# yang-song/score_sde_pytorch

Measured on NVIDIA H100. Metric: PC-sampler images/sec, NCSN++ CIFAR-10 1000-step VE, higher is better.
Workload: dtype f16 operands (11-bit significand, as tf32), f32 accumulate and activations

## Files before the change

### include/scoresde_b200.h

```cpp
#ifndef SCORESDE_B200_H_
#define SCORESDE_B200_H_

#ifdef __cplusplus
extern "C" {
#endif

#define B200_API __attribute__((visibility("default")))

B200_API const char* b200_last_error(void);
B200_API int b200_version(void);
B200_API int b200_device_sm_count(int* out);

B200_API int b200_upfirdn2d_f32(const float* x, const float* kernel_host, float* y,
                                int major, int in_h, int in_w, int minor, int kh, int kw,
                                int up_x, int up_y, int down_x, int down_y,
                                int pad_x0, int pad_x1, int pad_y0, int pad_y1, void* stream);

B200_API int b200_fused_bias_act_f32(const float* x, const float* b, const float* ref, float* y,
                                     long long n, int step_b, int size_b, int act, int grad,
                                     float alpha, float scale, void* stream);

B200_API int b200_groupnorm_nhwc_f32(const float* x1, int c1, const float* x2, int c2,
                                     const float* gamma, const float* beta, int batch, int hw, int groups,
                                     float eps, int silu, int round_tf32,
                                     float* stats_ws ,
                                     float* y, float* raw_or_null, void* stream);
B200_API int b200_softmax_rows_f32(const float* s, float* p, long long rows, int t, float scale,
                                   int round_tf32, void* stream);
B200_API int b200_randn_like_torch_f32(float* out, long long numel, unsigned long long seed,
                                       unsigned long long offset, unsigned long long* offset_inc_out,
                                       unsigned long long* offset_ws_dev , void* stream);

B200_API int b200_conv_nhwc_f32(const float* x1, int c1, const float* x2, int c2, int batch, int h, int w,
                                const float* w_packed, const float* bias, int c_out, int ksize,
                                const float* rowvec, long long rowvec_ld, const float* residual, float scale,
                                int round_tf32, float* out, int impl, void* stream);
B200_API int b200_conv_skip_nhwc_f32(const float* x, int c, const float* s1, int cs1, const float* s2, int cs2,
                                     int batch, int h, int w, const float* w_packed, const float* bias,
                                     const float* w_skip, const float* bias_skip, int c_out, const float* residual,
                                     float scale, int round_tf32, float* out, void* stream);
B200_API int b200_pack_conv_weight_f32(const float* w_oihw, float* w_packed, int c_out, int c_in, int ksize,
                                       int round_tf32, void* stream);
B200_API int b200_attention_core_f32(const float* qk, const float* vT, const float* w3, const float* bv,
                                     const float* b3, const float* x, float* out, double* qstats, int nimg,
                                     int t, int c, float out_scale, int operand_f16, void* stream);
B200_API int b200_gemm_nt_f32(const float* a, long long lda, int a_batch_rows, const float* w, long long ldw,
                              int w_batch_rows, int nbatch, int m, int n, int k, const float* bias,
                              int round_tf32, float* out, long long ldo, int impl, void* stream);

typedef struct b200_ncsnpp b200_ncsnpp_t;

typedef struct {
  int image_size, num_channels, nf, num_res_blocks;
  int num_levels;  int ch_mult[8];
  int num_attn_resolutions;  int attn_resolutions[8];
  int centered, scale_by_sigma, skip_rescale, conditional;
  int progressive_input;
  int fir_taps;  float fir_kernel[8];
  int precision;
  int keep_activations;
  int lanes;
  int cuda_core_head;
  int separate_groupnorm;
  int embedding_type;
  int naive_resample;
  int progressive;
  int pdl;
  int no_halo;
// ... 83 lines not shown
```

### score_sde_pytorch_b200/_lib.py

```python
import ctypes
import os
import threading

from . import build as _build

_LOCK = threading.Lock()
_LIB = None

c_void_p, c_int, c_ll, c_ull, c_float = (ctypes.c_void_p, ctypes.c_int, ctypes.c_longlong,
                                         ctypes.c_ulonglong, ctypes.c_float)
c_char_p = ctypes.c_char_p
P = ctypes.POINTER


class NcsnppConfig(ctypes.Structure):
  _fields_ = [('image_size', c_int), ('num_channels', c_int), ('nf', c_int), ('num_res_blocks', c_int),
              ('num_levels', c_int), ('ch_mult', c_int * 8),
              ('num_attn_resolutions', c_int), ('attn_resolutions', c_int * 8),
              ('centered', c_int), ('scale_by_sigma', c_int), ('skip_rescale', c_int), ('conditional', c_int),
              ('progressive_input', c_int),
              ('fir_taps', c_int), ('fir_kernel', c_float * 8),
              ('precision', c_int), ('keep_activations', c_int), ('lanes', c_int),
              ('cuda_core_head', c_int), ('separate_groupnorm', c_int),
              ('embedding_type', c_int), ('naive_resample', c_int), ('progressive', c_int), ('pdl', c_int),
# ... 7 lines not shown
              ('pa', P(c_float)), ('pb', P(c_float)), ('pc', P(c_float)),
              ('ca', P(c_float)), ('cb', P(c_float)), ('cc', P(c_float)),
              ('constraint', c_int), ('cm', P(c_float)), ('cs', P(c_float)),
              ('color_m', c_float * 9), ('color_minv', c_float * 9), ('noise_nhwc', c_int)]


SIGNATURES = {
  'b200_last_error': (c_char_p, []),
  'b200_version': (c_int, []),
  'b200_device_sm_count': (c_int, [P(c_int)]),
  'b200_upfirdn2d_f32': (c_int, [c_void_p, P(c_float), c_void_p] + [c_int] * 14 + [c_void_p]),
  'b200_fused_bias_act_f32': (c_int, [c_void_p, c_void_p, c_void_p, c_void_p, c_ll, c_int, c_int, c_int, c_int,
                                      c_float, c_float, c_void_p]),
  'b200_groupnorm_nhwc_f32': (c_int, [c_void_p, c_int, c_void_p, c_int, c_void_p, c_void_p, c_int, c_int, c_int,
                                      c_float, c_int, c_int, c_void_p, c_void_p, c_void_p, c_void_p]),
  'b200_softmax_rows_f32': (c_int, [c_void_p, c_void_p, c_ll, c_int, c_float, c_int, c_void_p]),
  'b200_randn_like_torch_f32': (c_int, [c_void_p, c_ll, c_ull, c_ull, P(c_ull), c_void_p, c_void_p]),
  'b200_conv_nhwc_f32': (c_int, [c_void_p, c_int, c_void_p, c_int, c_int, c_int, c_int, c_void_p, c_void_p, c_int,
                                 c_int, c_void_p, c_ll, c_void_p, c_float, c_int, c_void_p, c_int, c_void_p]),
  'b200_conv_skip_nhwc_f32': (c_int, [c_void_p, c_int, c_void_p, c_int, c_void_p, c_int, c_int, c_int, c_int, c_void_p,
                                      c_void_p, c_void_p, c_void_p, c_int, c_void_p, c_float, c_int, c_void_p, c_void_p]),
  'b200_attention_core_f32': (c_int, [c_void_p, c_void_p, c_void_p, c_void_p, c_void_p, c_void_p, c_void_p, c_void_p,
                                      c_int, c_int, c_int, c_float, c_int, c_void_p]),
  'b200_pack_conv_weight_f32': (c_int, [c_void_p, c_void_p, c_int, c_int, c_int, c_int, c_void_p]),
  'b200_gemm_nt_f32': (c_int, [c_void_p, c_ll, c_int, c_void_p, c_ll, c_int, c_int, c_int, c_int, c_int, c_void_p,
                               c_int, c_void_p, c_ll, c_int, c_void_p]),
  'b200_ncsnpp_create': (c_int, [P(NcsnppConfig), P(c_void_p)]),
  'b200_ncsnpp_destroy': (None, [c_void_p]),
  'b200_ncsnpp_num_params': (c_int, [c_void_p]),
  'b200_ncsnpp_param_info': (c_int, [c_void_p, c_int, c_char_p, c_int, P(c_ll), P(c_int)]),
  'b200_ncsnpp_weights_bytes': (c_ll, [c_void_p]),
  'b200_ncsnpp_bind_weights': (c_int, [c_void_p, c_void_p]),
  'b200_ncsnpp_load_param': (c_int, [c_void_p, c_int, c_void_p, c_void_p]),
  'b200_ncsnpp_num_ops': (c_ll, [c_void_p]),
  'b200_ncsnpp_op_info': (c_int, [c_void_p, c_ll, c_char_p, c_int, P(c_int), P(ctypes.c_double)]),
  'b200_ncsnpp_op_bytes': (c_int, [c_void_p, c_ll, P(ctypes.c_double)]),
  'b200_ncsnpp_profile_ops': (c_int, [c_void_p, c_void_p, c_void_p, c_int, c_void_p, c_void_p, c_void_p, c_ll]),
  'b200_ncsnpp_workspace_bytes': (c_ll, [c_void_p, c_int]),
  'b200_ncsnpp_bind_workspace': (c_int, [c_void_p, c_int, c_void_p, c_ll]),
  'b200_ncsnpp_forward': (c_int, [c_void_p, c_void_p, c_void_p, c_int, c_void_p, c_void_p]),
  'b200_ncsnpp_tap': (c_int, [c_void_p, c_int, c_void_p, c_ll, P(c_int), c_void_p]),
  'b200_ncsnpp_launches_per_forward': (c_ll, [c_void_p]),
  'b200_ncsnpp_jvp': (c_int, [c_void_p, c_void_p, c_void_p, c_int, c_void_p, c_void_p, c_void_p, c_void_p]),
  'b200_ncsnpp_tap_tangent': (c_int, [c_void_p, c_int, c_void_p, c_ll, P(c_int), c_void_p]),
  'b200_ncsnpp_profile_forward': (c_int, [c_void_p, c_void_p, c_void_p, c_int, c_void_p, c_void_p,
                                          P(c_float), P(ctypes.c_double), P(c_ll)]),
# ... 60 lines not shown
```

### score_sde_pytorch_b200/csrc/api.cu

```cuda
#include "kernels.h"
#include "../../include/scoresde_b200.h"
#include <cstring>

namespace b200 {
namespace { thread_local bool tl_pdl = false; }
bool pdl_active() { return tl_pdl; }
PdlScope::PdlScope(bool on) : prev(tl_pdl) { tl_pdl = on; }
PdlScope::~PdlScope() { tl_pdl = prev; }


static thread_local char g_err[1024] = "";

void set_error(const char* fmt, ...) {
  va_list ap;
  va_start(ap, fmt);
  vsnprintf(g_err, sizeof(g_err), fmt, ap);
  va_end(ap);
}
const char* last_error() { return g_err; }

}

using namespace b200;

// ... 107 lines not shown
  d.a3 = s1; d.C3 = cs1; d.a4 = s2; d.C4 = s2 ? cs2 : 0; d.w2 = w_skip;
  d.epi = ep;
  TcGemmPlan* pl = nullptr;
  if (int r = tc_gemm_plan_create(d, &pl)) return r;
  const int r = tc_gemm_launch(pl, static_cast<cudaStream_t>(stream));
  tc_gemm_plan_destroy(pl);
  return r;
}

int b200_attention_core_f32(const float* qk, const float* vT, const float* w3, const float* bv, const float* b3,
                            const float* x, float* out, double* qstats, int nimg, int t, int c, float out_scale,
                            int operand_f16, void* stream) {
  B200_REQUIRE(tc_attn_supported(t, c), "attention_core: only T=256, C=256 is implemented (got T=%d C=%d)", t, c);
  TcAttnDesc d; memset(&d, 0, sizeof(d));
  d.qk = qk; d.vT = vT; d.w3 = w3; d.bv = bv; d.b3 = b3; d.x = x; d.out = out; d.qstats = qstats;
  d.nimg = nimg; d.T = t; d.C = c; d.out_scale = out_scale; d.f16 = operand_f16 ? 1 : 0;
  TcAttnPlan* pl = nullptr;
  if (int r = tc_attn_plan_create(d, &pl)) return r;
  const int r = tc_attn_launch(pl, static_cast<cudaStream_t>(stream));
  tc_attn_plan_destroy(pl);
  return r;
}

int b200_gemm_nt_f32(const float* a, long long lda, int a_batch_rows, const float* w, long long ldw, int w_batch_rows,
                     int nbatch, int m, int n, int k, const float* bias, int round_tf32, float* out, long long ldo,
                     int impl, void* stream) {
  B200_REQUIRE(a && w && out && nbatch > 0, "gemm_nt: bad argument");
  cudaStream_t st = static_cast<cudaStream_t>(stream);
  Epilogue ep; memset(&ep, 0, sizeof(ep));
  ep.bias = bias; ep.scale = 1.f; ep.round_tf32 = round_tf32; ep.rows_per_img = m; ep.out = out; ep.ld_out = ldo;
  if (impl == 1 || impl == 2) {
    TcGemmDesc d; memset(&d, 0, sizeof(d));
    d.f16 = impl == 2;
    d.a1 = a; d.C1 = k; d.conv = 0; d.taps = 1; d.a_ld = lda; d.a_batch_rows = a_batch_rows;
    d.a_rows = a_batch_rows ? (long long)a_batch_rows * (nbatch - 1) + m : m;
    d.w = w; d.N_total = n; d.K_total = k; d.w_ld = ldw; d.w_batch_rows = w_batch_rows;
    d.w_rows = w_batch_rows ? (long long)w_batch_rows * (nbatch - 1) + n : n;
    d.nbatch = nbatch; d.M_per_batch = m; d.epi = ep;
    TcGemmPlan* pl = nullptr;
    if (int r = tc_gemm_plan_create(d, &pl)) return r;
    const int r = tc_gemm_launch(pl, st);
    tc_gemm_plan_destroy(pl);
    return r;
  }
  SimtConv s; memset(&s, 0, sizeof(s));
  s.x1 = a; s.C1 = k; s.ld1 = lda; s.in_scale = 1.f; s.H = m; s.W = 1; s.R = s.S = 1; s.stride = 1; s.pad = 0;
// ... 8 lines not shown
```

### score_sde_pytorch_b200/csrc/attn_tc.cuh

```cuda

constexpr int AT_T = 256, AT_C = 256;
template <bool F16>
struct AttnSmem {
  static constexpr int KB = F16 ? 4 : 8;
  static constexpr int BKA = F16 ? 64 : 32;
  static constexpr int PBUF = 0;
  static constexpr int RING = KB * 16384;
  static constexpr int STAGE_BYTES = A_STAGE_BYTES + 256 * 128;
  static constexpr int STAGES = F16 ? 3 : 2;
  static constexpr int BAR_OFFSET = RING + STAGES * STAGE_BYTES;
  static constexpr int TOTAL = BAR_OFFSET + 256 + 1024;
  static_assert(TOTAL <= 232448, "exceeds the 227 KB shared-memory limit of sm_90");
};

struct AttnParams {
  CUtensorMap tmQ, tmK, tmVT, tmW3;
  const float* bv;
  const float* b3;
  const float* x;
  float* out;
  double* qstats;
  float logit_scale;
  float out_scale;
  int nimg;
// ... 119 lines not shown
    for (int m = 1; m <= 2; m <<= 1) {
      suma += __shfl_xor_sync(0xffffffffu, suma, m);
      sumb += __shfl_xor_sync(0xffffffffu, sumb, m);
    }
    const float inva = 1.0f / suma, invb = 1.0f / sumb;
    fence_async_smem();
    wg_barrier(g);
    attn_phase<F16>(acc, 1, ring, pbuf, full_bar, empty_bar, stage, phase, g, lane);
    wg_barrier(g);
#pragma unroll
    for (int j = 0; j < 32; ++j) {
      const int ch = 8 * j + 2 * (lane & 3);
      const float2 t = __ldg(reinterpret_cast<const float2*>(p.bv + ch));
      pbuf_store2<F16>(pbuf, ra, ch, fmaf(acc[4 * j], inva, t.x), fmaf(acc[4 * j + 1], inva, t.y));
      pbuf_store2<F16>(pbuf, rb, ch, fmaf(acc[4 * j + 2], invb, t.x), fmaf(acc[4 * j + 3], invb, t.y));
    }
    fence_async_smem();
    wg_barrier(g);
    attn_phase<F16>(acc, 2, ring, pbuf, full_bar, empty_bar, stage, phase, g, lane);
    wg_barrier(g);
    Epilogue ep;
    ep.bias = p.b3; ep.rowvec = nullptr; ep.rowvec_ld = 0; ep.residual = p.x; ep.ld_res = AT_C; ep.per_img_div = nullptr;
    ep.div_stride = 0; ep.scale = p.out_scale; ep.round_tf32 = 0; ep.rows_per_img = AT_T; ep.out = p.out; ep.ld_out = AT_C;
    ep.out_nchw = 0; ep.n_valid = 0;
    const long long gm = (long long)b * AT_T + qh * BM + g * 64 + wq * 16;
    if (p.qstats) frag_rows<256, true, 0, true>(acc, ep, p.qstats, AT_C, gm, 16, 0, lane);
    else frag_rows<256, true, 0, false>(acc, ep, p.qstats, AT_C, gm, 16, 0, lane);
  }
}
```

### score_sde_pytorch_b200/csrc/common.cuh

```cuda
#pragma once
#include <cuda_runtime.h>
#include <cstdint>
#include <cstdio>
#include <cstdarg>
#include <string>
#include <utility>

namespace b200 {

void set_error(const char* fmt, ...);
const char* last_error();

#define B200_CHECK_CUDA(expr)                                                        \
  do {                                                                               \
    cudaError_t _e = (expr);                                                         \
    if (_e != cudaSuccess) {                                                         \
      (void)cudaGetLastError();  \
      ::b200::set_error("%s:%d: %s failed: %s", __FILE__, __LINE__, #expr,           \
                        cudaGetErrorString(_e));                                     \
      return 1;                                                                      \
    }                                                                                \
  } while (0)

#define B200_CHECK_LAUNCH()  B200_CHECK_CUDA(cudaGetLastError())
// ... 73 lines not shown
  cudaLaunchAttribute at = {};
  at.id = cudaLaunchAttributeProgrammaticStreamSerialization;
  at.val.programmaticStreamSerializationAllowed = 1;
  const bool on = pdl_active();
  cfg.attrs = on ? &at : nullptr; cfg.numAttrs = on ? 1 : 0;
  (void)cudaLaunchKernelEx(&cfg, kern, static_cast<KP>(args)...);
}

struct Epilogue {
  const float* bias;
  const float* rowvec;
  long long rowvec_ld;
  const float* residual;
  long long ld_res;
  const float* per_img_div;
  long long div_stride;
  float scale;
  int round_tf32;
  int rows_per_img;
  float* out;
  long long ld_out;
  int out_nchw;
  int n_valid;
};

}
```

### score_sde_pytorch_b200/csrc/engine.cu

```cuda
#include "kernels.h"
#include "../../include/scoresde_b200.h"
#include <cmath>
#include <cstring>
#include <functional>
#include <map>
#include <string>
#include <vector>

namespace b200 {
void tc_gemm_set_rowvec_ld(TcGemmPlan* p, long long ld);
}
using namespace b200;

namespace {

enum ModKind { M_FOURIER, M_LINEAR, M_CONV_IN, M_RESBLOCK, M_ATTN, M_PYR_DOWN, M_GN_OUT, M_CONV_OUT, M_COMBINE, M_DOWN, M_UP };
enum PackKind { PK_COPY = 0, PK_CONV = 1, PK_NIN = 2, PK_CONV_FLAT32 = 3, PK_CONV_PAD128 = 4 };

struct Param {
  std::string name;
  int ndim; long long shape[4];
  long long off, count;
  int pack, taps, O, I, round;
};
// ... 555 lines not shown
      d.a1 = A; d.C1 = K; d.conv = 0; d.taps = 1; d.a_rows = a_rows; d.a_ld = lda; d.a_batch_rows = a_batch_rows;
      d.w = Wm; d.N_total = N; d.K_total = K; d.w_rows = w_rows; d.w_ld = ldw; d.w_batch_rows = w_batch_rows;
      d.nbatch = nbatch; d.M_per_batch = M; d.qstats = qstats; d.epi = ep;
      d.f16 = om == 2;
      if (dry) return;
      TcGemmPlan* pl = nullptr;
      if (int r = tc_gemm_plan_create(d, &pl)) { rc = r; return; }
      e->tcplans.push_back(pl);
      name("gemm %dx(%dx%dx%d)%s [%s]", nbatch, M, N, K, residual ? " +res" : "", tc_gemm_form(pl));
      {
        const double es = om == 2 ? 2.0 : 4.0;
        next_bytes = (double)(a_batch_rows ? nbatch : 1) * M * K * es + (double)(w_batch_rows ? nbatch : 1) * N * K * es +
                     (double)nbatch * M * N * (round == 2 ? 2.0 : 4.0) + (residual ? (double)nbatch * M * N * 4.0 : 0.0);
      }
      op(1, [=](cudaStream_t st) { return tc_gemm_launch(pl, st); }, 0, 2.0 * nbatch * (double)M * N * K);
    } else {
      SimtConv s; memset(&s, 0, sizeof(s));
      s.x1 = A; s.C1 = K; s.ld1 = lda; s.in_scale = 1.f; s.H = M; s.W = 1; s.R = s.S = 1; s.stride = 1; s.pad = 0;
      s.OH = M; s.OW = 1; s.nbatch = nbatch; s.a_batched = a_batch_rows != 0; s.w = Wm; s.N = N;
      s.w_batch_stride = (long long)w_batch_rows * ldw; s.w_ld = ldw;
      ep.rows_per_img = M; s.epi = ep;
      op(1, [=](cudaStream_t st) { return launch_conv_simt(s, st); }, 1, 2.0 * nbatch * (double)M * N * K);
    }
  }

  const float* dense_all_ = nullptr;
  void tap(int idx, const Tensor& t) { if (!dry) e->taps[idx] = t; }

  bool lowc_ok(int C1, int C2, int Cout, int H, int taps) const {
    if (e->cfg.precision != 0 || e->sumC % 2 != 0) return false;
    SimtConv s; memset(&s, 0, sizeof(s));
    s.C1 = C1; s.C2 = C2; s.in_scale = 1.f; s.H = H; s.W = H; s.R = s.S = (taps == 9 ? 3 : 1); s.stride = 1; s.pad = (taps == 9 ? 1 : 0);
    s.OH = H; s.OW = H; s.nbatch = B; s.a_batched = 1; s.N = Cout; s.epi.ld_out = Cout; s.epi.ld_res = Cout;
    return conv_lowc_supported(s);
  }

  Tensor resblock(const Mod& m, Tensor& x1, Tensor& x2) {
    Tensor none;
    const int Cin = x1.C + x2.C, H = x1.H, Ho = m.up ? 2 * H : m.down ? H / 2 : H;
    const bool resample = m.up || m.down;
    const float inv_s2 = e->cfg.skip_rescale ? 1.0f / (float)std::sqrt(2.0) : 1.0f;
    const bool h1_f16 = om == 2 && m.tc0 && m.tc1 && fused_stats && (Ho * Ho) % 32 == 0 && (m.cout % 128 == 0);
    const int G0 = groups(Cin), G1 = groups(m.cout);
    const bool lc0 = lowc_gn && !m.tc0 && !resample && !x1.f16 && !x2.f16 && Cin % G0 == 0 && (Cin / G0) % 4 == 0 && x1.C % 4 == 0 &&
                     lowc_ok(x1.C, x2.C, m.cout, H, 9);
    const bool lc1 = lowc_gn && !m.tc1 && m.cout % G1 == 0 && (m.cout / G1) % 4 == 0 && lowc_ok(m.cout, 0, m.cout, Ho, 9);
// ... 88 lines not shown
    const float* bqkv = e->W(m.nb[0]);
    const float sc = 1.0f / std::sqrt((float)C);
    const long long BT = (long long)B * T;
    const int Bc = B;
    Tensor a = talloc(C, x.H, x.W);
    gn(x, none, m.gn0w, m.gn0b, 0, (tc || small) ? om : 0, a, nullptr);
    long long ob; float* O = nullptr;
    float* dO = nullptr;
    if (small) {
      long long qb; float* qkv = falloc(BT * 3 * C, &qb);
      gemm(true, a.p, C, BT, 0, Wqkv, C, 3LL * C, 0, 1, (int)BT, 3 * C, C, bqkv, nullptr, 0, 1.f, 0, qkv, 3 * C);
      tfree(a);
      O = falloc(BT * C, &ob);
      const int rnd = m.tc2 ? om : 0;
      if (!dry) { if (int r = launch_attn_small_configure(T, C)) { rc = r; } }
      name("attn_small T=%d C=%d", T, C);
      op(1, [=](cudaStream_t st) { return launch_attn_small(qkv, O, Bc, T, C, sc, rnd, st); }, 4);
      ffree(qkv, qb);
    } else {
      long long qkb, vtb, sb;
      float *dqk = nullptr, *dvT = nullptr, *dS = nullptr;
      float* qk = falloc2((long long)B * T * 2 * C, &qkb, &dqk);
      float* vT = falloc2((long long)B * C * T, &vtb, &dvT);
      gemm(tc, a.p, C, BT, 0 , Wqkv, C, 2LL * C, 0, 1, (int)BT, 2 * C, C, bqkv, nullptr, 0, 1.f, tc ? om : 0, qk, 2 * C);
      gemm(tc, wv, C, C, 0, a.p, C, BT, T, B, C, T, C, nullptr, nullptr, 0, 1.f, tc ? om : 0, vT, T, nullptr, 1 << 30);
      if (tan) {
        tan_op = true;
        gemm(tc, a.d, C, BT, 0, Wqkv, C, 2LL * C, 0, 1, (int)BT, 2 * C, C, nullptr, nullptr, 0, 1.f, tc ? om : 0, dqk, 2 * C);
        gemm(tc, wv, C, C, 0, a.d, C, BT, T, B, C, T, C, nullptr, nullptr, 0, 1.f, tc ? om : 0, dvT, T, nullptr, 1 << 30);
        tan_op = false;
      }
      tfree(a);
      if (om == 2 && !(tc && m.tc2 && tc_attn_supported(T, C))) {
        set_error("ncsnpp: fp16 operand mode needs the fused attention core (T=%d C=%d)", T, C); rc = 2; return Tensor();
      }
      if (tc && m.tc2 && tc_attn_supported(T, C) && !tan) {
        Tensor out = talloc(C, x.H, x.W);
        if (fused_stats) out.qs = qalloc(C);
        if (!dry) {
          TcAttnDesc d; memset(&d, 0, sizeof(d));
          d.qk = qk; d.vT = vT; d.w3 = e->W(m.nw[3]); d.bv = bqkv + 2 * C; d.b3 = e->W(m.nb[3]); d.x = x.p; d.out = out.p;
          d.qstats = out.qs; d.nimg = B; d.T = T; d.C = C; d.out_scale = inv_s2; d.f16 = om == 2;
          TcAttnPlan* pl = nullptr;
          if (int r = tc_attn_plan_create(d, &pl)) { rc = r; return Tensor(); }
          e->attnplans.push_back(pl);
          name("attention core T=%d C=%d (QK^T, softmax, PV, NIN_3 +res) [fused]", T, C);
          next_bytes = (double)B * T * C * ((om == 2 ? 2.0 : 4.0) * 3 + 8.0) + (double)C * C * (om == 2 ? 2.0 : 4.0);
          op(1, [=](cudaStream_t st) { return tc_attn_launch(pl, st); }, 0, 2.0 * B * T * ((double)T * C * 2 + (double)C * C));
        }
        ffree(qk, qkb); ffree(vT, vtb);
        return out;
      }
      float* S = falloc2(BT * T, &sb, &dS);
// ... 914 lines not shown
```

### score_sde_pytorch_b200/csrc/gemm_tc.cu

```cuda
#include "kernels.h"
#include <cuda.h>
#include <cudaTypedefs.h>
#include <cuda_fp16.h>
#include "wgmma.cuh"
#include <mutex>
#include <cstdlib>
#include <cstring>

namespace b200 {

namespace {

constexpr int BM = 128;
constexpr int BKE = 32;
constexpr int A_STAGE_BYTES = BM * BKE * 4;

constexpr int HALO_XS = 4;
constexpr int HALO_X_BYTES = 40 * 1024;
constexpr int HALO_WS = 4;

struct TcParams {
  CUtensorMap tmA1, tmA2, tmW;
  CUtensorMap tmA3, tmA4, tmW2;
  CUtensorMap tmH1, tmH2;
// ... 92 lines not shown
__device__ __forceinline__ void wg_barrier(int g) { asm volatile("bar.sync %0, 128;" ::"r"(g + 1) : "memory"); }

template <int BN>
struct SmemLayout {
  static constexpr int STAGES = BN == 256 ? 4 : 6;
  static constexpr int B_STAGE_BYTES = BN * BKE * 4;
  static constexpr int STAGE_BYTES = A_STAGE_BYTES + B_STAGE_BYTES;
  static constexpr int RING_BYTES = STAGES * STAGE_BYTES;
  static constexpr int HALO_BYTES = HALO_XS * HALO_X_BYTES + HALO_WS * A_STAGE_BYTES;
  static constexpr int BAR_OFFSET = BN == 256 && HALO_BYTES > RING_BYTES ? HALO_BYTES : RING_BYTES;
  static constexpr int TOTAL = BAR_OFFSET + 256 + 1024;
  static_assert(TOTAL <= 232448, "exceeds the 227 KB shared-memory limit of sm_90");
  static_assert(BN != 256 || STAGES >= HALO_XS, "the halo copies use the first HALO_XS stage barriers");
};

template <int BN, bool RES, int MODE, bool STATS>
__device__ __forceinline__ void frag_rows(const float (&d)[BN / 2], const Epilogue& e, double* qstats, int n_total,
                                          long long gm, int rows_valid, int n0, int lane) {
  const int ra = lane >> 2, rb = ra + 8;
  const bool va = ra < rows_valid, vb = rb < rows_valid;
  const int img = rows_valid > 0 ? (int)gm / e.rows_per_img : 0;
  const float* rv = e.rowvec ? e.rowvec + (long long)img * e.rowvec_ld : nullptr;
  const float scale = e.scale;
#pragma unroll
  for (int j = 0; j < BN / 8; ++j) {
    const int col = n0 + 8 * j + 2 * (lane & 3);
    float2 ad = make_float2(0.f, 0.f);
    if (e.bias) ad = __ldg(reinterpret_cast<const float2*>(e.bias + col));
    if (rv) { const float2 t = __ldg(reinterpret_cast<const float2*>(rv + col)); ad.x += t.x; ad.y += t.y; }
    float o0 = d[4 * j] + ad.x, o1 = d[4 * j + 1] + ad.y, o2 = d[4 * j + 2] + ad.x, o3 = d[4 * j + 3] + ad.y;
    if (RES) {
      if (va) { const float2 r = __ldg(reinterpret_cast<const float2*>(e.residual + (gm + ra) * e.ld_res + col)); o0 += r.x; o1 += r.y; }
      if (vb) { const float2 r = __ldg(reinterpret_cast<const float2*>(e.residual + (gm + rb) * e.ld_res + col)); o2 += r.x; o3 += r.y; }
    }
    o0 *= scale; o1 *= scale; o2 *= scale; o3 *= scale;
    if (MODE == 1) { o0 = round_tf32(o0); o1 = round_tf32(o1); o2 = round_tf32(o2); o3 = round_tf32(o3); }
    if (MODE == 2) {
      uint16_t* oh = reinterpret_cast<uint16_t*>(e.out);
      if (va) *reinterpret_cast<uint32_t*>(oh + (gm + ra) * e.ld_out + col) = pack_half2(o0, o1);
      if (vb) *reinterpret_cast<uint32_t*>(oh + (gm + rb) * e.ld_out + col) = pack_half2(o2, o3);
    } else {
      if (va) *reinterpret_cast<float2*>(e.out + (gm + ra) * e.ld_out + col) = make_float2(o0, o1);
      if (vb) *reinterpret_cast<float2*>(e.out + (gm + rb) * e.ld_out + col) = make_float2(o2, o3);
    }
    if (STATS) {
      float s = (va ? o0 + o1 : 0.f) + (vb ? o2 + o3 : 0.f);
      float q = (va ? fmaf(o0, o0, o1 * o1) : 0.f) + (vb ? fmaf(o2, o2, o3 * o3) : 0.f);
#pragma unroll
      for (int m = 4; m <= 16; m <<= 1) { s += __shfl_xor_sync(0xffffffffu, s, m); q += __shfl_xor_sync(0xffffffffu, q, m); }
      s += __shfl_xor_sync(0xffffffffu, s, 1); q += __shfl_xor_sync(0xffffffffu, q, 1);
      if ((lane & ~2) == 0 && rows_valid > 0) {
        double* qd = qstats + ((long long)img * (n_total >> 2) + (col >> 2)) * 2;
        atomicAdd(qd, (double)s); atomicAdd(qd + 1, (double)q);
      }
    }
  }
}
template <int BN>
__device__ __forceinline__ void frag_rows_dispatch(const float (&d)[BN / 2], const Epilogue& e, double* qstats, int n_total,
                                                   long long gm, int rows_valid, int n0, int lane) {
  const int mode = e.round_tf32;
  const bool has_res = e.residual != nullptr, stats = qstats != nullptr;
#define B200_ROWF(R, M) do { if (stats) frag_rows<BN, R, M, true>(d, e, qstats, n_total, gm, rows_valid, n0, lane); \
                             else frag_rows<BN, R, M, false>(d, e, qstats, n_total, gm, rows_valid, n0, lane); } while (0)
  if (has_res) { if (mode == 0) B200_ROWF(true, 0); else if (mode == 1) B200_ROWF(true, 1); else B200_ROWF(true, 2); }
  else { if (mode == 0) B200_ROWF(false, 0); else if (mode == 1) B200_ROWF(false, 1); else B200_ROWF(false, 2); }
#undef B200_ROWF
}

template <bool RES, int MODE, bool STATS>
__device__ __forceinline__ void frag_swap(const float (&d)[128], const Epilogue& e, double* qstats, int n_total,
                                          int c0, long long pix0, int img, int lane) {
  const int ca = c0 + (lane >> 2), cb = ca + 8;
  const float adda = (e.bias ? __ldg(e.bias + ca) : 0.f) + (e.rowvec ? __ldg(e.rowvec + img * e.rowvec_ld + ca) : 0.f);
  const float addb = (e.bias ? __ldg(e.bias + cb) : 0.f) + (e.rowvec ? __ldg(e.rowvec + img * e.rowvec_ld + cb) : 0.f);
  const float scale = e.scale;
  float sa = 0.f, qa = 0.f, sb = 0.f, qb = 0.f;
#pragma unroll
// ... 10 lines not shown
      if (MODE == 2) {
        uint16_t h;
        asm("cvt.rn.f16.f32 %0, %1;" : "=h"(h) : "f"(o[i]));
        reinterpret_cast<uint16_t*>(e.out)[pix * e.ld_out + ch] = h;
      } else e.out[pix * e.ld_out + ch] = o[i];
    }
    if (STATS) {
      sa += o[0] + o[1]; qa = fmaf(o[0], o[0], fmaf(o[1], o[1], qa));
      sb += o[2] + o[3]; qb = fmaf(o[2], o[2], fmaf(o[3], o[3], qb));
    }
  }
  if (STATS) {
#pragma unroll
    for (int m = 1; m <= 8; m <<= 1) {
      sa += __shfl_xor_sync(0xffffffffu, sa, m); qa += __shfl_xor_sync(0xffffffffu, qa, m);
      sb += __shfl_xor_sync(0xffffffffu, sb, m); qb += __shfl_xor_sync(0xffffffffu, qb, m);
    }
    if ((lane & 15) == 0) {
      double* qd = qstats + ((long long)img * (n_total >> 2) + (ca >> 2)) * 2;
      atomicAdd(qd, (double)sa); atomicAdd(qd + 1, (double)qa);
      qd = qstats + ((long long)img * (n_total >> 2) + (cb >> 2)) * 2;
      atomicAdd(qd, (double)sb); atomicAdd(qd + 1, (double)qb);
    }
  }
}

template <int BN, bool F16>
__device__ __forceinline__ void gemm_tc_consumer(const TcParams& p, uint8_t* smem, uint64_t* full_bar, uint64_t* empty_bar,
                                                 uint64_t* wfull_bar, uint64_t* wempty_bar, int g, int wq, int lane) {
  using L = SmemLayout<BN>;
  const int kiters = (p.kchunks1 + p.kchunks2) * p.taps + p.kchunks3 + p.kchunks4;
  const Epilogue& e = p.epi;
  uint32_t stage = 0, phase = 0, ws = 0, wphase = 0;
  for (int tile = blockIdx.x; tile < p.total_tiles; tile += gridDim.x) {
    float acc[BN / 2];
    if (BN == 256 && p.halo) {
      const uint32_t wring = smem_u32(smem + HALO_XS * HALO_X_BYTES);
      int it = 0, pend_ws = -1, pend_x = -1;
      for (int src = 0; src < 4; ++src) {
        const int nch = src == 0 ? p.kchunks1 : src == 1 ? p.kchunks2 : src == 2 ? p.kchunks3 : p.kchunks4;
        const int ncopies = src < 2 ? 3 * nch : nch, ntap = src < 2 ? 3 : 1;
        for (int c = 0; c < ncopies; ++c) {
          mbar_wait(&full_bar[stage], phase);
          const uint32_t sx = smem_u32(smem + stage * HALO_X_BYTES);
          for (int dhi = 0; dhi < ntap; ++dhi, ++it) {
            mbar_wait(&wfull_bar[ws], wphase);
// ... 31 lines not shown
      if (lane == 0 && pend >= 0) mbar_arrive(&empty_bar[pend]);
    }

    const int rw = g * 64 + wq * 16;
    if constexpr (BN == 256) {
      if (p.swap) {
        const int c0 = (int)(tile % p.tiles_n) * 128 + rw;
        const int pix0 = (tile / p.tiles_n) * 256;
        const int img = pix0 / e.rows_per_img;
        if (e.out_nchw) {
          const float dv = e.per_img_div ? __ldg(e.per_img_div + img * e.div_stride) : 1.f;
          const int hw = e.rows_per_img, pix_in_img = (int)(pix0 - (long long)img * hw);
#pragma unroll
          for (int h = 0; h < 2; ++h) {
            const int co = c0 + (lane >> 2) + 8 * h;
            if (co < e.n_valid) {
              const float add = e.bias ? __ldg(e.bias + co) : 0.f;
              float* dst = e.out + ((long long)img * e.n_valid + co) * hw + pix_in_img + 2 * (lane & 3);
#pragma unroll
              for (int j = 0; j < 32; ++j)
                *reinterpret_cast<float2*>(dst + 8 * j) = make_float2((acc[4 * j + 2 * h] + add) / dv, (acc[4 * j + 2 * h + 1] + add) / dv);
            }
          }
        } else {
          const int mode = e.round_tf32;
          const bool has_res = e.residual != nullptr, stats = p.qstats != nullptr;
#define B200_SWAPF(R, M) do { if (stats) frag_swap<R, M, true>(acc, e, p.qstats, p.N_total, c0, pix0, img, lane); \
                              else frag_swap<R, M, false>(acc, e, p.qstats, p.N_total, c0, pix0, img, lane); } while (0)
          if (has_res) { if (mode == 0) B200_SWAPF(true, 0); else if (mode == 1) B200_SWAPF(true, 1); else B200_SWAPF(true, 2); }
          else { if (mode == 0) B200_SWAPF(false, 0); else if (mode == 1) B200_SWAPF(false, 1); else B200_SWAPF(false, 2); }
#undef B200_SWAPF
        }
        continue;
      }
    }
    const int nt = (int)(tile % p.tiles_n);
    const int mg = tile / p.tiles_n;
    const int b = (int)(mg / p.tiles_m_per_batch);
    const int mt = (int)(mg % p.tiles_m_per_batch);
    const int row0 = mt * BM + rw;
    const int rows_valid = min(16, max(0, p.M_per_batch - row0));
    frag_rows_dispatch<BN>(acc, e, p.qstats, p.N_total, (long long)b * p.M_per_batch + row0, rows_valid, nt * BN, lane);
  }
}

template <int BN>
// ... 202 lines not shown
  if (d.taps != 1 && d.taps != 9) return fail("only 1x1 and 3x3 filters");
  if (d.conv) {
    if (d.nbatch != 1) return fail("conv mode is unbatched");
    if (d.stride > 2) return fail("stride must be 1 or 2");
    if (d.stride == 2 && d.a2) return fail("strided conv is single-source");
    const int HW = d.H * d.W;
    if (HW >= BM) {
      if (d.W >= BM) { if (d.W % BM) return fail("image width does not tile 128 pixels"); }
      else if ((BM % d.W) || (d.H % (BM / d.W))) return fail("image rows do not tile 128 pixels");
    } else if (BM % HW) return fail("image size does not divide 128 pixels");
  } else {
    if (d.nbatch > 1 && (d.M_per_batch % BM)) return fail("batched gemm needs M_per_batch % 128 == 0");
    if (d.a_ld % (d.f16 ? 8 : 4)) return fail("A row pitch must be a multiple of 16 bytes");
  }
  if (d.a3) {
    if (!d.conv || d.stride == 2 || !d.w2) return fail("extra 1x1 phase needs a stride-1 convolution and its weights");
    if (d.C3 % bke || d.C3 <= 0 || (d.a4 && d.C4 % bke)) return fail("extra-phase channel counts must be multiples of 32 (tf32) / 64 (f16)");
  }
  if (d.epi.out_nchw) {
    if (!(d.conv && d.N_total == 128 && d.epi.n_valid > 0 && d.epi.n_valid <= 32 && (d.H * d.W) % 256 == 0 && (d.W <= BM || d.W % BM == 0) && d.stride != 2 &&
          !d.qstats && !d.epi.residual && !d.epi.rowvec && d.epi.round_tf32 == 0))
      return fail("NCHW head needs a 128-row padded weight tile, HW % 256 == 0 and a plain epilogue");
  } else if (d.epi.per_img_div) return fail("per-image divisor only with the NCHW head epilogue");
  if ((d.qstats || d.epi.rowvec) && !(d.epi.rows_per_img % 32 == 0 || d.epi.rows_per_img == 16)) return fail("per-image epilogue terms need rows_per_img % 32 == 0 or == 16");
  if (d.epi.ld_out % 4 || (d.epi.residual && d.epi.ld_res % 4)) return fail("output pitch must be a multiple of 4 elements");
  if (d.epi.round_tf32 == 2 && d.epi.ld_out % 8) return fail("fp16 output pitch must be a multiple of 8 elements");
  return true;
}

int tc_gemm_plan_create(const TcGemmDesc& d, TcGemmPlan** out) {
  const char* why = nullptr;
  B200_REQUIRE(tc_gemm_supported(d, &why), "gemm_tc: unsupported shape: %s", why ? why : "?");
  if (int r = tc_configure()) return r;
  TcGemmPlan* pl = new TcGemmPlan();
  TcParams& p = pl->prm;
  memset(&p, 0, sizeof(p));
  pl->bn = (d.N_total % 256 == 0) ? 256 : 128;
  p.conv = d.conv; p.H = d.conv ? d.H : 1; p.W = d.conv ? d.W : 1; p.taps = d.taps;
  p.S = d.taps == 9 ? 3 : 1; p.pad = (d.taps == 9 && !d.valid_pad) ? 1 : 0;
  p.stride = d.stride == 2 ? 2 : 1;
  p.f16 = d.f16 ? 1 : 0;

  const bool f16 = d.f16 != 0;
  const int bke = f16 ? 64 : BKE;
  const uint64_t es = f16 ? 2 : 4;
  p.bke = bke;
  {
    const long long Mtot = (long long)d.nimg * d.H * d.W;
    const bool halo_geom = d.taps == 9 && p.pad == 1 && (d.W == 16 || d.W == 32) && (d.Hin == 0 || d.Hin == d.H) &&
                           (d.Win == 0 || d.Win == d.W);
    const bool can_swap = d.conv && p.stride == 1 && (d.N_total % 256 != 0 || d.taps == 1 || halo_geom) && (d.H * d.W) % 256 == 0 &&
                          (d.W <= BM || d.W % BM == 0) && Mtot % 256 == 0 && d.epi.rows_per_img % 256 == 0;
    p.swap = can_swap ? 1 : 0;
    if (d.epi.out_nchw && !p.swap) { delete pl; B200_REQUIRE(false, "gemm_tc: the NCHW head needs the swapped-operand form"); }
    if (p.swap) pl->bn = 256;
    p.qstats = d.qstats;
    const int tmb = d.conv ? 1 : (d.M_per_batch + BM - 1) / BM;
    const long long m_tiles = d.conv ? (Mtot + BM - 1) / BM : (long long)d.nbatch * tmb;
    const long long n_tiles = d.N_total % 256 == 0 ? d.N_total / 256 : d.N_total / 128;
    if (!p.swap && pl->bn == 256 && m_tiles * n_tiles <= num_sms() / 2) pl->bn = 128;
  }
  p.kchunks1 = d.C1 / bke; p.kchunks2 = d.a2 ? d.C2 / bke : 0; p.C1 = d.C1;
  p.N_total = d.N_total; p.tiles_n = p.swap ? d.N_total / 128 : d.N_total / pl->bn;
  p.a_batch_rows = d.a_batch_rows; p.w_batch_rows = d.w_batch_rows;
  p.epi = d.epi;

  int rc = 0;
  if (d.conv) {
    const int HW = d.H * d.W;
    const long long M = (long long)d.nimg * HW;
    p.nbatch = 1; p.M_per_batch = (int)M; p.tiles_m_per_batch = p.swap ? (int)(M / 256) : (int)((M + BM - 1) / BM);
    uint32_t box[4];
    if (HW >= BM) { box[1] = std::min(d.W, BM); box[2] = BM / box[1]; box[3] = 1; }
    else { box[1] = d.W; box[2] = d.H; box[3] = BM / HW; }
    box[0] = (uint32_t)bke;
    const uint32_t estr[4] = {1, (uint32_t)p.stride, (uint32_t)p.stride, 1};
    box[1] *= p.stride; box[2] *= p.stride;
// ... 72 lines not shown
    p.tmW2 = p.tmW;
    if (d.a3) {
      const uint64_t K3 = (uint64_t)d.C3 + (d.a4 ? d.C4 : 0);
      uint64_t dims2[2] = {K3, (uint64_t)d.N_total};
      uint64_t str2[1] = {K3 * es};
      rc = encode_map(&p.tmW2, d.w2, 2, dims2, str2, box, nullptr, f16);
      if (rc) { delete pl; return rc; }
    }
  }
  p.total_tiles = (long long)p.nbatch * p.tiles_m_per_batch * p.tiles_n;
  *out = pl;
  return 0;
}

void tc_gemm_plan_destroy(TcGemmPlan* p) { delete p; }
const char* tc_gemm_form(const TcGemmPlan* p) {
  if (p->prm.swap) return p->prm.halo ? "swap-halo" : "swap";
  return p->bn == 256 ? "single256" : "single128";
}
void tc_gemm_set_rowvec_ld(TcGemmPlan* p, long long ld) { p->prm.epi.rowvec_ld = ld; }
void tc_gemm_set_head(TcGemmPlan* p, float* out_nchw, const float* per_img_div, long long div_stride) {
  p->prm.epi.out = out_nchw; p->prm.epi.per_img_div = per_img_div; p->prm.epi.div_stride = div_stride;
}
struct TcAttnPlan { AttnParams prm; bool f16; };

bool tc_attn_supported(int T, int C) { return T == AT_T && C == AT_C; }

int tc_attn_plan_create(const TcAttnDesc& d, TcAttnPlan** out) {
  B200_REQUIRE(tc_attn_supported(d.T, d.C), "attn_tc: only T=256, C=256 (got T=%d C=%d)", d.T, d.C);
  B200_REQUIRE(d.qk && d.vT && d.w3 && d.bv && d.b3 && d.x && d.out && d.nimg > 0, "attn_tc: null argument");
  if (int r = tc_configure()) return r;
  TcAttnPlan* pl = new TcAttnPlan();
  AttnParams& p = pl->prm;
  memset(&p, 0, sizeof(p));
  pl->f16 = d.f16 != 0;
  const bool f16 = pl->f16;
  const uint64_t es = f16 ? 2 : 4;
  const uint32_t bka = f16 ? 64 : 32;
  int rc = 0;
  {
    uint64_t dims[2] = {(uint64_t)2 * AT_C, (uint64_t)d.nimg * AT_T};
    uint64_t str[1] = {(uint64_t)2 * AT_C * es};
    uint32_t boxq[2] = {bka, (uint32_t)BM}, boxk[2] = {bka, 256};
    rc = encode_map(&p.tmQ, d.qk, 2, dims, str, boxq, nullptr, f16);
    if (!rc) rc = encode_map(&p.tmK, d.qk, 2, dims, str, boxk, nullptr, f16);
  }
// ... 55 lines not shown
```

### score_sde_pytorch_b200/csrc/kernels.h

```cpp
#pragma once
#include <cuda_runtime.h>
#include <cstdint>
#include <algorithm>
#include "common.cuh"

namespace b200 {

int launch_gn_quad_stats(const float* x, int C, int B, int HW, double* qsums, cudaStream_t st, bool qsums_zeroed = false);
int launch_gn_apply(const float* x1, int C1, const float* x2, int C2, const double* q1, const double* q2,
                    const float* gamma, const float* beta, int B, int HW, int G, float eps, int act,
                    int round_out, float* y, float* raw, cudaStream_t st, int x1_f16 = 0);
int launch_gn_generic(const float* x1, int C1, const float* x2, int C2, const float* gamma, const float* beta, int B, int HW, int G,
                      float eps, int act, int round_out, float* y, float* raw, float* mr_ws, cudaStream_t st);
long long gn_generic_workspace_floats(int B, int HW, int G);
int launch_gn_coeff(int C1, int C2, const double* q1, const double* q2, const float* gamma, const float* beta, int B, int HW,
                    int G, float eps, float* scale, float* shift, cudaStream_t st);
int launch_upfirdn2d(const float* x, const float* kernel_host, float* y, int major, int in_h, int in_w,
                     int minor, int kh, int kw, int up_x, int up_y, int down_x, int down_y,
                     int pad_x0, int pad_x1, int pad_y0, int pad_y1, int round_out, cudaStream_t st);
int launch_fused_bias_act(const float* x, const float* b, const float* ref, float* y, long long n,
                          int step_b, int size_b, int act, int grad, float alpha, float scale,
                          cudaStream_t st);
int launch_softmax_rows(const float* s, float* p, long long rows, int T, float scale, int round_out,
                        cudaStream_t st);
// ... 49 lines not shown
  int conv;
  int H, W, nimg;
  int taps;
  int stride;
  int valid_pad;
  int Hin, Win;
  long long a_rows;
  long long a_ld;
  int a_batch_rows;
  const float* w; int N_total; int K_total; long long w_rows;
  long long w_ld;
  int w_batch_rows;
  int nbatch; int M_per_batch;
  const float* a3; int C3; const float* a4; int C4; const float* w2;
  int f16;
  int no_halo;
  double* qstats;
  Epilogue epi;
};
int tc_gemm_plan_create(const TcGemmDesc& d, TcGemmPlan** out);
void tc_gemm_plan_destroy(TcGemmPlan* p);
int tc_gemm_launch(const TcGemmPlan* p, cudaStream_t st);
bool tc_gemm_supported(const TcGemmDesc& d, const char** why);
struct TcAttnPlan;
struct TcAttnDesc {
  const float* qk;
  const float* vT;
  const float* w3;
  const float* bv;
  const float* b3;
  const float* x;
  float* out;
  double* qstats;
  int nimg, T, C;
  float out_scale;
  int f16;
};
bool tc_attn_supported(int T, int C);
int tc_attn_plan_create(const TcAttnDesc& d, TcAttnPlan** out);
void tc_attn_plan_destroy(TcAttnPlan* p);
int tc_attn_launch(const TcAttnPlan* p, cudaStream_t st);
void tc_gemm_set_head(TcGemmPlan* p, float* out_nchw, const float* per_img_div, long long div_stride);
const char* tc_gemm_form(const TcGemmPlan* p);

struct PhiloxMap {
  unsigned long long seed;
// ... 39 lines not shown
```

Measured before the change: 8.188.

## Fuse attention Q|K and transposed V projections into one tensor-core GEMM launch

Replaces the two separate GEMMs that produce the Q|K matrix and the transposed V matrix with a single 1x1-convolution tensor-core GEMM over the concatenated qkv weight. A new epilogue writes the first 2C channels pixel-major and the last C channels channel-major, using in-register lane transposes and 8-wide stores. The change also batches residual loads in the row epilogue and defers qstats atomics to one set per lane after the loop. This removes one kernel launch and one extra read of the activations per attention block, at the cost of a more complex epilogue with extra shuffles and support checks that restrict it to the swapped-operand form.

```diff
diff --git a/include/scoresde_b200.h b/include/scoresde_b200.h
--- a/include/scoresde_b200.h
+++ b/include/scoresde_b200.h
@@ -44,6 +44,8 @@
 B200_API int b200_attention_core_f32(const float* qk, const float* vT, const float* w3, const float* bv,
                                      const float* b3, const float* x, float* out, double* qstats, int nimg,
                                      int t, int c, float out_scale, int operand_f16, void* stream);
+B200_API int b200_attention_proj_f32(const float* a, const float* w_qkv, const float* b_qk, int nimg, int h, int w,
+                                     int c, float* qk, float* vT, int operand_f16, void* stream);
 B200_API int b200_gemm_nt_f32(const float* a, long long lda, int a_batch_rows, const float* w, long long ldw,
                               int w_batch_rows, int nbatch, int m, int n, int k, const float* bias,
                               int round_tf32, float* out, long long ldo, int impl, void* stream);
diff --git a/score_sde_pytorch_b200/_lib.py b/score_sde_pytorch_b200/_lib.py
--- a/score_sde_pytorch_b200/_lib.py
+++ b/score_sde_pytorch_b200/_lib.py
@@ -53,6 +53,8 @@
                                       c_void_p, c_void_p, c_void_p, c_int, c_void_p, c_float, c_int, c_void_p, c_void_p]),
   'b200_attention_core_f32': (c_int, [c_void_p, c_void_p, c_void_p, c_void_p, c_void_p, c_void_p, c_void_p, c_void_p,
                                       c_int, c_int, c_int, c_float, c_int, c_void_p]),
+  'b200_attention_proj_f32': (c_int, [c_void_p, c_void_p, c_void_p, c_int, c_int, c_int, c_int, c_void_p, c_void_p, c_int,
+                                      c_void_p]),
   'b200_pack_conv_weight_f32': (c_int, [c_void_p, c_void_p, c_int, c_int, c_int, c_int, c_void_p]),
   'b200_gemm_nt_f32': (c_int, [c_void_p, c_ll, c_int, c_void_p, c_ll, c_int, c_int, c_int, c_int, c_int, c_void_p,
                                c_int, c_void_p, c_ll, c_int, c_void_p]),
diff --git a/score_sde_pytorch_b200/csrc/api.cu b/score_sde_pytorch_b200/csrc/api.cu
--- a/score_sde_pytorch_b200/csrc/api.cu
+++ b/score_sde_pytorch_b200/csrc/api.cu
@@ -153,6 +153,17 @@
   return r;
 }
 
+int b200_attention_proj_f32(const float* a, const float* w_qkv, const float* b_qk, int nimg, int h, int w, int c, float* qk,
+                            float* vT, int operand_f16, void* stream) {
+  B200_REQUIRE(a && w_qkv && qk && vT && nimg > 0, "attention_proj: bad argument");
+  B200_REQUIRE(tc_attn_proj_supported(h, w, c), "attention_proj: needs H*W %% 256 == 0, W <= 128, C %% 128 == 0 (got %dx%d, C=%d)", h, w, c);
+  TcGemmPlan* pl = nullptr;
+  if (int r = tc_gemm_plan_create(tc_attn_proj_desc(a, w_qkv, b_qk, nimg, h, w, c, operand_f16 ? 1 : 0, qk, vT), &pl)) return r;
+  const int r = tc_gemm_launch(pl, static_cast<cudaStream_t>(stream));
+  tc_gemm_plan_destroy(pl);
+  return r;
+}
+
 int b200_gemm_nt_f32(const float* a, long long lda, int a_batch_rows, const float* w, long long ldw, int w_batch_rows,
                      int nbatch, int m, int n, int k, const float* bias, int round_tf32, float* out, long long ldo,
                      int impl, void* stream) {
diff --git a/score_sde_pytorch_b200/csrc/attn_tc.cuh b/score_sde_pytorch_b200/csrc/attn_tc.cuh
--- a/score_sde_pytorch_b200/csrc/attn_tc.cuh
+++ b/score_sde_pytorch_b200/csrc/attn_tc.cuh
@@ -165,7 +165,7 @@
     Epilogue ep;
     ep.bias = p.b3; ep.rowvec = nullptr; ep.rowvec_ld = 0; ep.residual = p.x; ep.ld_res = AT_C; ep.per_img_div = nullptr;
     ep.div_stride = 0; ep.scale = p.out_scale; ep.round_tf32 = 0; ep.rows_per_img = AT_T; ep.out = p.out; ep.ld_out = AT_C;
-    ep.out_nchw = 0; ep.n_valid = 0;
+    ep.out_nchw = 0; ep.n_valid = 0; ep.out_t = nullptr; ep.t_from = 0;
     const long long gm = (long long)b * AT_T + qh * BM + g * 64 + wq * 16;
     if (p.qstats) frag_rows<256, true, 0, true>(acc, ep, p.qstats, AT_C, gm, 16, 0, lane);
     else frag_rows<256, true, 0, false>(acc, ep, p.qstats, AT_C, gm, 16, 0, lane);
diff --git a/score_sde_pytorch_b200/csrc/common.cuh b/score_sde_pytorch_b200/csrc/common.cuh
--- a/score_sde_pytorch_b200/csrc/common.cuh
+++ b/score_sde_pytorch_b200/csrc/common.cuh
@@ -119,6 +119,8 @@
   long long ld_out;
   int out_nchw;
   int n_valid;
+  float* out_t;
+  int t_from;
 };
 
 }
diff --git a/score_sde_pytorch_b200/csrc/engine.cu b/score_sde_pytorch_b200/csrc/engine.cu
--- a/score_sde_pytorch_b200/csrc/engine.cu
+++ b/score_sde_pytorch_b200/csrc/engine.cu
@@ -601,6 +601,18 @@
       ep.rows_per_img = M; s.epi = ep;
       op(1, [=](cudaStream_t st) { return launch_conv_simt(s, st); }, 1, 2.0 * nbatch * (double)M * N * K);
     }
+  }
+
+  void attn_proj(const float* a, const float* w_qkv, const float* b_qk, int H, int W, int C, float* qk, float* vT) {
+    const TcGemmDesc d = tc_attn_proj_desc(a, w_qkv, b_qk, B, H, W, C, om == 2, qk, vT);
+    if (dry) return;
+    TcGemmPlan* pl = nullptr;
+    if (int r = tc_gemm_plan_create(d, &pl)) { rc = r; return; }
+    e->tcplans.push_back(pl);
+    name("attn proj q|k|vT %d->%d @%d [%s]", C, 3 * C, H, tc_gemm_form(pl));
+    const double es = om == 2 ? 2.0 : 4.0, px = (double)B * H * W;
+    next_bytes = px * C * es + px * 3.0 * C * es + 3.0 * C * C * es;
+    op(1, [=](cudaStream_t st) { return tc_gemm_launch(pl, st); }, 0, 2.0 * px * 3.0 * C * C);
   }
 
   const float* dense_all_ = nullptr;
@@ -735,13 +747,18 @@
       float *dqk = nullptr, *dvT = nullptr, *dS = nullptr;
       float* qk = falloc2((long long)B * T * 2 * C, &qkb, &dqk);
       float* vT = falloc2((long long)B * C * T, &vtb, &dvT);
-      gemm(tc, a.p, C, BT, 0 , Wqkv, C, 2LL * C, 0, 1, (int)BT, 2 * C, C, bqkv, nullptr, 0, 1.f, tc ? om : 0, qk, 2 * C);
-      gemm(tc, wv, C, C, 0, a.p, C, BT, T, B, C, T, C, nullptr, nullptr, 0, 1.f, tc ? om : 0, vT, T, nullptr, 1 << 30);
-      if (tan) {
-        tan_op = true;
-        gemm(tc, a.d, C, BT, 0, Wqkv, C, 2LL * C, 0, 1, (int)BT, 2 * C, C, nullptr, nullptr, 0, 1.f, tc ? om : 0, dqk, 2 * C);
-        gemm(tc, wv, C, C, 0, a.d, C, BT, T, B, C, T, C, nullptr, nullptr, 0, 1.f, tc ? om : 0, dvT, T, nullptr, 1 << 30);
-        tan_op = false;
+      if (tc && tc_attn_proj_supported(x.H, x.W, C)) {
+        attn_proj(a.p, Wqkv, bqkv, x.H, x.W, C, qk, vT);
+        if (tan) { tan_op = true; attn_proj(a.d, Wqkv, nullptr, x.H, x.W, C, dqk, dvT); tan_op = false; }
+      } else {
+        gemm(tc, a.p, C, BT, 0 , Wqkv, C, 2LL * C, 0, 1, (int)BT, 2 * C, C, bqkv, nullptr, 0, 1.f, tc ? om : 0, qk, 2 * C);
+        gemm(tc, wv, C, C, 0, a.p, C, BT, T, B, C, T, C, nullptr, nullptr, 0, 1.f, tc ? om : 0, vT, T, nullptr, 1 << 30);
+        if (tan) {
+          tan_op = true;
+          gemm(tc, a.d, C, BT, 0, Wqkv, C, 2LL * C, 0, 1, (int)BT, 2 * C, C, nullptr, nullptr, 0, 1.f, tc ? om : 0, dqk, 2 * C);
+          gemm(tc, wv, C, C, 0, a.d, C, BT, T, B, C, T, C, nullptr, nullptr, 0, 1.f, tc ? om : 0, dvT, T, nullptr, 1 << 30);
+          tan_op = false;
+        }
       }
       tfree(a);
       if (om == 2 && !(tc && m.tc2 && tc_attn_supported(T, C))) {
diff --git a/score_sde_pytorch_b200/csrc/gemm_tc.cu b/score_sde_pytorch_b200/csrc/gemm_tc.cu
--- a/score_sde_pytorch_b200/csrc/gemm_tc.cu
+++ b/score_sde_pytorch_b200/csrc/gemm_tc.cu
@@ -138,16 +138,28 @@
   const int img = rows_valid > 0 ? (int)gm / e.rows_per_img : 0;
   const float* rv = e.rowvec ? e.rowvec + (long long)img * e.rowvec_ld : nullptr;
   const float scale = e.scale;
+  const int qh = (lane >> 1) & 1, qidx = ((lane >> 2) << 1) | (lane & 1);
+  float qs0 = 0.f, qq0 = 0.f, qs1 = 0.f, qq1 = 0.f;
+  constexpr int RG = 8;
+  float2 resa[RG], resb[RG];
 #pragma unroll
   for (int j = 0; j < BN / 8; ++j) {
     const int col = n0 + 8 * j + 2 * (lane & 3);
+    if (RES && j % RG == 0) {
+#pragma unroll
+      for (int g = 0; g < RG; ++g) {
+        const int cg = col + 8 * g;
+        resa[g] = va ? __ldg(reinterpret_cast<const float2*>(e.residual + (gm + ra) * e.ld_res + cg)) : make_float2(0.f, 0.f);
+        resb[g] = vb ? __ldg(reinterpret_cast<const float2*>(e.residual + (gm + rb) * e.ld_res + cg)) : make_float2(0.f, 0.f);
+      }
+    }
     float2 ad = make_float2(0.f, 0.f);
     if (e.bias) ad = __ldg(reinterpret_cast<const float2*>(e.bias + col));
     if (rv) { const float2 t = __ldg(reinterpret_cast<const float2*>(rv + col)); ad.x += t.x; ad.y += t.y; }
     float o0 = d[4 * j] + ad.x, o1 = d[4 * j + 1] + ad.y, o2 = d[4 * j + 2] + ad.x, o3 = d[4 * j + 3] + ad.y;
     if (RES) {
-      if (va) { const float2 r = __ldg(reinterpret_cast<const float2*>(e.residual + (gm + ra) * e.ld_res + col)); o0 += r.x; o1 += r.y; }
-      if (vb) { const float2 r = __ldg(reinterpret_cast<const float2*>(e.residual + (gm + rb) * e.ld_res + col)); o2 += r.x; o3 += r.y; }
+      if (va) { const float2 r = resa[j % RG]; o0 += r.x; o1 += r.y; }
+      if (vb) { const float2 r = resb[j % RG]; o2 += r.x; o3 += r.y; }
     }
     o0 *= scale; o1 *= scale; o2 *= scale; o3 *= scale;
     if (MODE == 1) { o0 = round_tf32(o0); o1 = round_tf32(o1); o2 = round_tf32(o2); o3 = round_tf32(o3); }
@@ -165,11 +177,14 @@
 #pragma unroll
       for (int m = 4; m <= 16; m <<= 1) { s += __shfl_xor_sync(0xffffffffu, s, m); q += __shfl_xor_sync(0xffffffffu, q, m); }
       s += __shfl_xor_sync(0xffffffffu, s, 1); q += __shfl_xor_sync(0xffffffffu, q, 1);
-      if ((lane & ~2) == 0 && rows_valid > 0) {
-        double* qd = qstats + ((long long)img * (n_total >> 2) + (col >> 2)) * 2;
-        atomicAdd(qd, (double)s); atomicAdd(qd + 1, (double)q);
-      }
-    }
+      if (j == qidx) { qs0 = s; qq0 = q; }
+      if (j == qidx + 16) { qs1 = s; qq1 = q; }
+    }
+  }
+  if (STATS && rows_valid > 0) {
+    double* qd = qstats + ((long long)img * (n_total >> 2) + (n0 >> 2) + 2 * qidx + qh) * 2;
+    atomicAdd(qd, (double)qs0); atomicAdd(qd + 1, (double)qq0);
+    if (BN / 8 > 16) { atomicAdd(qd + 64, (double)qs1); atomicAdd(qd + 65, (double)qq1); }
   }
 }
 template <int BN>
@@ -226,6 +241,69 @@
       qd = qstats + ((long long)img * (n_total >> 2) + (cb >> 2)) * 2;
       atomicAdd(qd, (double)sb); atomicAdd(qd + 1, (double)qb);
     }
+  }
+}
+
+template <int N, int E>
+__device__ __forceinline__ void lane_transpose(float (&v)[N * E], int r, int s) {
+#pragma unroll
+  for (int b = 1; b < N; b <<= 1) {
+    const bool up = (r & b) != 0;
+#pragma unroll
+    for (int k = 0; k < N; ++k) {
+      if (k & b) continue;
+#pragma unroll
+      for (int x = 0; x < E; ++x) {
+        const float got = __shfl_xor_sync(0xffffffffu, up ? v[E * k + x] : v[E * (k | b) + x], s * b);
+        if (up) v[E * k + x] = got; else v[E * (k | b) + x] = got;
+      }
+    }
+  }
+}
+__device__ __forceinline__ void store8(float* base, long long idx, const float (&v)[8], int mode) {
+  if (mode == 2) {
+    const uint4 u = make_uint4(pack_half2(v[0], v[1]), pack_half2(v[2], v[3]), pack_half2(v[4], v[5]), pack_half2(v[6], v[7]));
+    *reinterpret_cast<uint4*>(reinterpret_cast<uint16_t*>(base) + idx) = u;
+  } else {
+    float w[8];
+#pragma unroll
+    for (int k = 0; k < 8; ++k) w[k] = mode == 1 ? round_tf32(v[k]) : v[k];
+    *reinterpret_cast<float4*>(base + idx) = make_float4(w[0], w[1], w[2], w[3]);
+    *reinterpret_cast<float4*>(base + idx + 4) = make_float4(w[4], w[5], w[6], w[7]);
+  }
+}
+
+__device__ __forceinline__ void frag_swap_pix(const float (&d)[128], const Epilogue& e, int c0, long long pix0, int lane) {
+  const int r = lane >> 2, q = lane & 3;
+  const float adda = e.bias ? __ldg(e.bias + c0 + r) : 0.f, addb = e.bias ? __ldg(e.bias + c0 + 8 + r) : 0.f;
+  const float scale = e.scale;
+  const long long row = pix0 + 8 * (r >> 2) + 2 * q + (r & 1);
+  const int ch = c0 + 8 * ((r >> 1) & 1);
+#pragma unroll
+  for (int j = 0; j < 32; j += 2) {
+    float v[8];
+#pragma unroll
+    for (int k = 0; k < 8; ++k) v[k] = (d[4 * j + k] + ((k & 2) ? addb : adda)) * scale;
+    lane_transpose<8, 1>(v, r, 4);
+    store8(e.out, (row + 8 * j) * e.ld_out + ch, v, e.round_tf32);
+  }
+}
+__device__ __forceinline__ void frag_swap_t(const float (&d)[128], const Epilogue& e, int n_t, int ct, int pix, int img, int lane) {
+  const int q = lane & 3;
+  const long long ia = ((long long)img * n_t + ct + (lane >> 2)) * e.rows_per_img + pix, ib = ia + 8LL * e.rows_per_img;
+  const float scale = e.scale;
+#pragma unroll
+  for (int j = 0; j < 32; j += 4) {
+    float va[8], vb[8];
+#pragma unroll
+    for (int jj = 0; jj < 4; ++jj) {
+#pragma unroll
+      for (int s = 0; s < 2; ++s) { va[2 * jj + s] = d[4 * (j + jj) + s] * scale; vb[2 * jj + s] = d[4 * (j + jj) + 2 + s] * scale; }
+    }
+    lane_transpose<4, 2>(va, q, 1);
+    lane_transpose<4, 2>(vb, q, 1);
+    store8(e.out_t, ia + 8 * (j + q), va, e.round_tf32);
+    store8(e.out_t, ib + 8 * (j + q), vb, e.round_tf32);
   }
 }
 
@@ -303,6 +381,9 @@
                 *reinterpret_cast<float2*>(dst + 8 * j) = make_float2((acc[4 * j + 2 * h] + add) / dv, (acc[4 * j + 2 * h + 1] + add) / dv);
             }
           }
+        } else if (e.out_t) {
+          if (c0 >= e.t_from) frag_swap_t(acc, e, p.N_total - e.t_from, c0 - e.t_from, (int)(pix0 - (long long)img * e.rows_per_img), img, lane);
+          else frag_swap_pix(acc, e, c0, pix0, lane);
         } else {
           const int mode = e.round_tf32;
           const bool has_res = e.residual != nullptr, stats = p.qstats != nullptr;
@@ -551,6 +632,11 @@
           !d.qstats && !d.epi.residual && !d.epi.rowvec && d.epi.round_tf32 == 0))
       return fail("NCHW head needs a 128-row padded weight tile, HW % 256 == 0 and a plain epilogue");
   } else if (d.epi.per_img_div) return fail("per-image divisor only with the NCHW head epilogue");
+  if (d.epi.out_t) {
+    if (!(d.conv && d.taps == 1 && d.epi.t_from > 0 && d.epi.t_from % 128 == 0 && d.epi.t_from < d.N_total &&
+          d.epi.ld_out >= d.epi.t_from && !d.qstats && !d.epi.residual && !d.epi.rowvec && !d.epi.out_nchw))
+      return fail("channel-major output needs a 1x1 convolution, a 128-aligned split and a plain epilogue");
+  }
   if ((d.qstats || d.epi.rowvec) && !(d.epi.rows_per_img % 32 == 0 || d.epi.rows_per_img == 16)) return fail("per-image epilogue terms need rows_per_img % 32 == 0 or == 16");
   if (d.epi.ld_out % 4 || (d.epi.residual && d.epi.ld_res % 4)) return fail("output pitch must be a multiple of 4 elements");
   if (d.epi.round_tf32 == 2 && d.epi.ld_out % 8) return fail("fp16 output pitch must be a multiple of 8 elements");
@@ -582,6 +668,7 @@
                           (d.W <= BM || d.W % BM == 0) && Mtot % 256 == 0 && d.epi.rows_per_img % 256 == 0;
     p.swap = can_swap ? 1 : 0;
     if (d.epi.out_nchw && !p.swap) { delete pl; B200_REQUIRE(false, "gemm_tc: the NCHW head needs the swapped-operand form"); }
+    if (d.epi.out_t && !p.swap) { delete pl; B200_REQUIRE(false, "gemm_tc: a channel-major output needs the swapped-operand form"); }
     if (p.swap) pl->bn = 256;
     p.qstats = d.qstats;
     const int tmb = d.conv ? 1 : (d.M_per_batch + BM - 1) / BM;
@@ -700,6 +787,17 @@
 void tc_gemm_set_head(TcGemmPlan* p, float* out_nchw, const float* per_img_div, long long div_stride) {
   p->prm.epi.out = out_nchw; p->prm.epi.per_img_div = per_img_div; p->prm.epi.div_stride = div_stride;
 }
+bool tc_attn_proj_supported(int H, int W, int C) { return (H * W) % 256 == 0 && W <= BM && C % 128 == 0; }
+TcGemmDesc tc_attn_proj_desc(const float* a, const float* w_qkv, const float* b_qk, int nimg, int H, int W, int C, int f16,
+                             float* qk, float* vT) {
+  TcGemmDesc d; memset(&d, 0, sizeof(d));
+  d.a1 = a; d.C1 = C; d.conv = 1; d.H = H; d.W = W; d.nimg = nimg; d.taps = 1; d.nbatch = 1;
+  d.w = w_qkv; d.N_total = 3 * C; d.K_total = C; d.w_rows = 3LL * C; d.f16 = f16;
+  Epilogue& ep = d.epi;
+  ep.bias = b_qk; ep.scale = 1.f; ep.round_tf32 = f16 ? 2 : 1; ep.rows_per_img = H * W;
+  ep.out = qk; ep.ld_out = 2 * C; ep.out_t = vT; ep.t_from = 2 * C;
+  return d;
+}
 struct TcAttnPlan { AttnParams prm; bool f16; };
 
 bool tc_attn_supported(int T, int C) { return T == AT_T && C == AT_C; }
diff --git a/score_sde_pytorch_b200/csrc/kernels.h b/score_sde_pytorch_b200/csrc/kernels.h
--- a/score_sde_pytorch_b200/csrc/kernels.h
+++ b/score_sde_pytorch_b200/csrc/kernels.h
@@ -95,6 +95,9 @@
 void tc_gemm_plan_destroy(TcGemmPlan* p);
 int tc_gemm_launch(const TcGemmPlan* p, cudaStream_t st);
 bool tc_gemm_supported(const TcGemmDesc& d, const char** why);
+bool tc_attn_proj_supported(int H, int W, int C);
+TcGemmDesc tc_attn_proj_desc(const float* a, const float* w_qkv, const float* b_qk, int nimg, int H, int W, int C, int f16,
+                             float* qk, float* vT);
 struct TcAttnPlan;
 struct TcAttnDesc {
   const float* qk;
```

Measured after the change: 8.467 (median of 6 runs). 1.03x the previous value.
